# deu439/ARFlow

Hardware: AMD Instinct MI355X
Metric: image-pairs/sec fwd+bwd, PWCLite 384x640 bs=8 (higher is better)
Workload: dtype f32; 1 GPU; pwclite_uflow+uflow_loss, 384x640 pairs, batch 8 per GPU, fwd(both directions)+loss+bwd+allreduce+Adam; global_batch=8, parallelism=dp1, step_start=seeded weights + fresh Adam state, restored before every step, loss_finite=True

## Files before the change

arflow_amd/csrc/splitbf16.hpp:

```cpp
#pragma once
#include <array>

#include "common.hpp"

namespace splitbf16 {
typedef __bf16 bf16x8 __attribute__((ext_vector_type(8)));
typedef float f32x16 __attribute__((ext_vector_type(16)));

struct Split {
  __bf16 p[3];
  __device__ __forceinline__ explicit Split(float v) {
    p[0] = (__bf16)v;
    const float r1 = v - (float)p[0];
    p[1] = (__bf16)r1;
    p[2] = (__bf16)(r1 - (float)p[1]);
  }
};

template <class F>
__device__ __forceinline__ void split8(const F& value, bf16x8 (&o)[3]) {
#pragma unroll
  for (int e = 0; e < 8; ++e) {
    const Split s(value(e));
    o[0][e] = s.p[0], o[1][e] = s.p[1], o[2][e] = s.p[2];
  }
}

__device__ __forceinline__ int acc_channel(int i, int hh) { return (i & 3) + 8 * (i >> 2) + 4 * hh; }

__device__ __forceinline__ void acc_zero(f32x16& a) {
#pragma unroll
  for (int i = 0; i < 16; ++i) a[i] = 0.f;
}
template <class T, int N>
__device__ __forceinline__ void acc_zero(T (&a)[N]) {
#pragma unroll
  for (int s = 0; s < N; ++s) acc_zero(a[s]);
}

inline int tiles32(int n) { return (n + 31) / 32; }
constexpr int MAX_KT = 2;

struct TilePart { int kt, count, first; };
inline std::array<TilePart, 2> split_tiles(int nkt, int max_kt) {
  const int chunks = (nkt + max_kt - 1) / max_kt, base = nkt / chunks, extra = nkt % chunks;
  return {{{base + 1, extra, 0}, {base, chunks - extra, extra * (base + 1)}}};
}

template <auto KERNEL>
inline int allow_dynamic_lds(int bytes) {
  static bool attr_set = false;
  if (!attr_set) {
    const hipError_t e = hipFuncSetAttribute(reinterpret_cast<const void*>(KERNEL), hipFuncAttributeMaxDynamicSharedMemorySize, bytes);
    if (e != hipSuccess) return af_hip_status(e);
    attr_set = true;
  }
  return ARFLOW_OK;
}
}
```

arflow_amd/csrc/splitconv_wgrad.hip:

```cpp
#include <climits>
#include <cstdint>

#include "splitbf16.hpp"

namespace {
using namespace splitbf16;
typedef unsigned u32x4 __attribute__((ext_vector_type(4)));

constexpr int G = 8;
constexpr int DY_CS = 3 * G + 1;
constexpr int X_CS = 9 * G + 1;
constexpr int XH_CS = 9 * G + 1;
constexpr int MAX_ROWS = 128;
constexpr int MIN_ROWS = 4;
constexpr int WANT_WG = 1024;

template <int KT>
struct Lds {
  static constexpr int DY = 0;
  static constexpr int X = KT * 32 * DY_CS * 16;
  static constexpr int XH = X + 32 * X_CS * 16;
  static constexpr int BYTES = XH + 32 * XH_CS * 4;
};

__device__ __forceinline__ unsigned bf16_bits(__bf16 b) { return (unsigned)__builtin_bit_cast(unsigned short, b); }

struct Run {
  float4 a, b;
  float l, r;
};
template <bool VEC>
__device__ __forceinline__ void load_run(const float* __restrict__ row, int col0, int W, bool valid, Run& o) {
  const float4 z = make_float4(0.f, 0.f, 0.f, 0.f);
  if (VEC) {
    const bool in0 = col0 < W, in1 = col0 + 4 < W;
    const float4 t0 = *reinterpret_cast<const float4*>(row + (in0 ? col0 : 0));
    const float4 t1 = *reinterpret_cast<const float4*>(row + (in1 ? col0 + 4 : 0));
    o.a = valid && in0 ? t0 : z;
    o.b = valid && in1 ? t1 : z;
  } else {
    float t[8];
#pragma unroll
    for (int e = 0; e < 8; ++e) t[e] = row[min(col0 + e, W - 1)];
#pragma unroll
    for (int e = 0; e < 8; ++e) t[e] = (valid && col0 + e < W) ? t[e] : 0.f;
    o.a = make_float4(t[0], t[1], t[2], t[3]);
    o.b = make_float4(t[4], t[5], t[6], t[7]);
  }
}

struct Plan {
  int GW, SG, nstrips, RPC, nrb, nct, nkt, kchunks;
  long chunks;
};
inline bool shape_ok(int N, int C, int K, int H, int W) {
  return N > 0 && C > 0 && K > 0 && H > 0 && W > 0 && (long)N * C * H * W <= INT_MAX && (long)N * K * H * W <= INT_MAX &&
         (long)9 * K * C <= INT_MAX;
}
inline Plan make_plan(int N, int C, int K, int H, int W) {
  Plan p;
  p.GW = (W + 7) / 8;
  const int ns = (p.GW + G - 1) / G;
  p.SG = 2 * ((p.GW + 2 * ns - 1) / (2 * ns));
  p.nstrips = (p.GW + p.SG - 1) / p.SG;
  p.nct = tiles32(C), p.nkt = tiles32(K), p.kchunks = (p.nkt + MAX_KT - 1) / MAX_KT;
  const long units = (long)p.nct * p.kchunks * N * p.nstrips;
  const long want = (WANT_WG + units - 1) / units;
  int rpc = (int)((H + want - 1) / want);
  if (rpc < MIN_ROWS) rpc = MIN_ROWS;
  if (rpc > MAX_ROWS) rpc = MAX_ROWS;
  if (rpc > H) rpc = H;
  p.RPC = rpc;
  p.nrb = (H + rpc - 1) / rpc;
  p.chunks = (long)N * p.nstrips * p.nrb;
  return p;
}

template <int KT, bool VEC>
__global__ __launch_bounds__(192 * KT, VEC && KT == 2 ? 3 : 2) void splitconv_wgrad_kernel(const float* __restrict__ x, long x_bs,
                                                                             const float* __restrict__ dy, long dy_bs,
                                                                             float* __restrict__ ws, int C, int K, int H, int W,
                                                                             int kt_first, int kcnt, int nct, int nstrips, int SG,
                                                                             int nrb, int RPC) {
  constexpr int NT = 192 * KT;
  using L = Lds<KT>;
  extern __shared__ __align__(16) unsigned char lds[];
  unsigned* const xh = reinterpret_cast<unsigned*>(lds + L::XH);
  const int tid = threadIdx.x, lane = tid & 63, wv = __builtin_amdgcn_readfirstlane(tid >> 6);
  const int r32 = lane & 31, hh = lane >> 5;
  const int ktl = wv / 3, tr = wv - 3 * ktl;
  const int b = blockIdx.x;
  const int ct = b % nct, kc = (b / nct) % kcnt, chunk = b / (nct * kcnt);
  const int rb = chunk % nrb, strip = (chunk / nrb) % nstrips, n = chunk / (nrb * nstrips);
  const int kt0 = kt_first + kc * KT;
  const int h0 = rb * RPC, h1 = min(H, h0 + RPC);
  const int GW = (W + 7) >> 3, g0 = strip * SG, gcount = min(SG, GW - g0), nsteps = (gcount + 1) >> 1;
  const long HWl = (long)H * W;
  const float* const xn = x + (long)n * x_bs;
  const float* const dyn = dy + (long)n * dy_bs;

  constexpr int NX = 32 * G, NITEM = NX + KT * 32 * G, NSLOT = (NITEM + NT - 1) / NT;
  Run pf[NSLOT];
  const auto fetch = [&](int yx, int ydy) __attribute__((always_inline)) {
#pragma unroll
    for (int j = 0; j < NSLOT; ++j) {
      const int i = tid + j * NT;
      if (i < NX) {
        const int cl = i / G, g = i - cl * G;
        const int c = ct * 32 + cl, col0 = (g0 + g) * 8;
        const bool valid = yx >= 0 && yx < H && c < C && g < gcount;
        const float* row = xn + (valid ? (long)c * HWl + (long)yx * W : 0);
        load_run<VEC>(row, col0, W, valid, pf[j]);
        const float vl = row[max(col0 - 1, 0)], vr = row[min(col0 + 8, W - 1)];
        pf[j].l = (valid && col0 > 0) ? vl : 0.f;
        pf[j].r = (valid && col0 + 8 < W) ? vr : 0.f;
      } else if (i < NITEM && ydy >= 0) {
        const int kl = (i - NX) / G, g = (i - NX) - kl * G;
        const int k = kt0 * 32 + kl, col0 = (g0 + g) * 8;
        const bool valid = k < K && g < gcount;
        const float* row = dyn + (valid ? (long)k * HWl + (long)ydy * W : 0);
        load_run<VEC>(row, col0, W, valid, pf[j]);
      }
    }
  };
  const auto commit = [&](int yx, int ydy) __attribute__((always_inline)) {
    const int slot = (yx + 3) % 3;
#pragma unroll
    for (int j = 0; j < NSLOT; ++j) {
      const int i = tid + j * NT;
      if (i < NX) {
        const int cl = i / G, g = i - cl * G;
        const float v[8] = {pf[j].a.x, pf[j].a.y, pf[j].a.z, pf[j].a.w, pf[j].b.x, pf[j].b.y, pf[j].b.z, pf[j].b.w};
        bf16x8 o[3];
#pragma unroll
        for (int e = 0; e < 8; ++e) {
          const Split s(v[e]);
          o[0][e] = s.p[0], o[1][e] = s.p[1], o[2][e] = s.p[2];
        }
        const Split sl(pf[j].l), sr(pf[j].r);
#pragma unroll
        for (int p = 0; p < 3; ++p) {
          const int at = (slot * 3 + p) * G + g;
          *reinterpret_cast<bf16x8*>(lds + L::X + (cl * X_CS + at) * 16) = o[p];
          xh[cl * XH_CS + at] = (bf16_bits(sl.p[p]) << 16) | bf16_bits(sr.p[p]);
        }
      } else if (i < NITEM && ydy >= 0) {
        const int kl = (i - NX) / G, g = (i - NX) - kl * G;
        const float v[8] = {pf[j].a.x, pf[j].a.y, pf[j].a.z, pf[j].a.w, pf[j].b.x, pf[j].b.y, pf[j].b.z, pf[j].b.w};
        bf16x8 o[3];
#pragma unroll
        for (int e = 0; e < 8; ++e) {
          const Split s(v[e]);
          o[0][e] = s.p[0], o[1][e] = s.p[1], o[2][e] = s.p[2];
        }
#pragma unroll
        for (int p = 0; p < 3; ++p) *reinterpret_cast<bf16x8*>(lds + L::DY + (kl * DY_CS + p * G + g) * 16) = o[p];
      }
    }
  };

  f32x16 tot[3];
  acc_zero(tot);

  const unsigned char* const a_base = lds + L::DY + ((ktl * 32 + r32) * DY_CS + hh) * 16;
  fetch(h0 - 1, -1);
  commit(h0 - 1, -1);
  fetch(h0, -1);
  commit(h0, -1);
  fetch(h0 + 1, h0);
  for (int h = h0; h < h1; ++h) {
    if (h > h0) __syncthreads();
    commit(h + 1, h);
    __syncthreads();
    fetch(h + 2, h + 1 < h1 ? h + 1 : -1);
    const int slot = (h + tr + 2) % 3;
    const unsigned char* const b_base = lds + L::X + (r32 * X_CS + slot * 3 * G + hh) * 16;
    const unsigned* const bh_base = xh + r32 * XH_CS + slot * 3 * G + hh;
    f32x16 acc[3];
    acc_zero(acc);
    const auto x_frags = [&](int p, int t, bf16x8 (&bs)[3]) __attribute__((always_inline)) {
      const u32x4 d = *reinterpret_cast<const u32x4*>(b_base + (p * G + 2 * t) * 16);
      const unsigned nb = bh_base[p * G + 2 * t];
      const unsigned m1 = __builtin_amdgcn_alignbit(d.y, d.x, 16), m2 = __builtin_amdgcn_alignbit(d.z, d.y, 16),
                     m3 = __builtin_amdgcn_alignbit(d.w, d.z, 16);
      const u32x4 lo = {__builtin_amdgcn_alignbit(d.x, nb, 16), m1, m2, m3};
      const u32x4 hi = {m1, m2, m3, __builtin_amdgcn_alignbit(nb, d.w, 16)};
      bs[0] = __builtin_bit_cast(bf16x8, lo);
      bs[1] = __builtin_bit_cast(bf16x8, d);
      bs[2] = __builtin_bit_cast(bf16x8, hi);
    };
#pragma unroll 1
    for (int t = 0; t < nsteps; ++t) {
      bf16x8 a[3], bs[3];
#pragma unroll
      for (int p = 0; p < 3; ++p) a[p] = *reinterpret_cast<const bf16x8*>(a_base + (p * G + 2 * t) * 16);
#pragma unroll
      for (int p = 2; p >= 0; --p) {
        x_frags(p, t, bs);
#pragma unroll
        for (int pa = 2 - p; pa >= (p == 0 ? 1 : 0); --pa)
#pragma unroll
          for (int s = 0; s < 3; ++s) acc[s] = __builtin_amdgcn_mfma_f32_32x32x16_bf16(a[pa], bs[s], acc[s], 0, 0, 0);
      }
    }
#pragma unroll 1
    for (int t = 0; t < nsteps; ++t) {
      bf16x8 bs[3];
      const bf16x8 a0 = *reinterpret_cast<const bf16x8*>(a_base + (2 * t) * 16);
      x_frags(0, t, bs);
#pragma unroll
      for (int s = 0; s < 3; ++s) acc[s] = __builtin_amdgcn_mfma_f32_32x32x16_bf16(a0, bs[s], acc[s], 0, 0, 0);
    }
#pragma unroll
    for (int s = 0; s < 3; ++s) tot[s] = tot[s] + acc[s];
  }
  const int c = ct * 32 + r32;
  if (c < C) {
#pragma unroll
    for (int s = 0; s < 3; ++s) {
      float* const wt = ws + ((long)chunk * 9 + (tr * 3 + s)) * K * C;
#pragma unroll
      for (int i = 0; i < 16; ++i) {
        const int k = 32 * (kt0 + ktl) + acc_channel(i, hh);
        if (k < K) wt[(long)k * C + c] = tot[s][i];
      }
    }
  }
}

__global__ __launch_bounds__(256) void splitconv_wgrad_finish_kernel(const float* __restrict__ ws, float* __restrict__ dw, int K,
                                                                       int C, int chunks) {
  const int KC = K * C, e = blockIdx.x * 256 + threadIdx.x;
  if (e >= 9 * KC) return;
  const int tap = e / KC, kc = e - tap * KC;
  double s = 0.0;
  for (int ch = 0; ch < chunks; ++ch) s += (double)ws[(long)ch * 9 * KC + e];
  dw[(long)kc * 9 + tap] = (float)s;
}

template <int KT, bool VEC>
int launch(const float* x, long x_bs, const float* dy, long dy_bs, float* ws, int C, int K, int H, int W, int kt_first, int kcnt,
           const Plan& p, hipStream_t st) {
  using L = Lds<KT>;
  if (const int rc = allow_dynamic_lds<&splitconv_wgrad_kernel<KT, VEC>>(L::BYTES)) return rc;
  const long grid = p.chunks * kcnt * p.nct;
  if (grid > INT_MAX) return ARFLOW_ESHAPE;
  hipLaunchKernelGGL((splitconv_wgrad_kernel<KT, VEC>), dim3((unsigned)grid), dim3(192 * KT), L::BYTES, st, x, x_bs, dy, dy_bs, ws, C, K,
                     H, W, kt_first, kcnt, p.nct, p.nstrips, p.SG, p.nrb, p.RPC);
  return af_launch_status();
}
}

extern "C" long arflow_splitconv_wgrad_ws_bytes(int N, int C, int K, int H, int W) {
  if (!shape_ok(N, C, K, H, W)) return ARFLOW_ESHAPE;
  const Plan p = make_plan(N, C, K, H, W);
  if (p.chunks > INT_MAX) return ARFLOW_ESHAPE;
  return p.chunks * 9 * K * C * 4;
}

extern "C" int arflow_splitconv_wgrad(const float* x, long x_bstride, const float* dy, long dy_bstride, float* dw, void* ws, int N,
                                      int C, int K, int H, int W, arflow_stream_t stream) {
  af_clear_stale_error();
  AF_REQUIRE_PTR(x);
  AF_REQUIRE_PTR(dy);
  AF_REQUIRE_PTR(dw);
  AF_REQUIRE_PTR(ws);
  AF_REQUIRE(shape_ok(N, C, K, H, W), ARFLOW_ESHAPE);
  AF_REQUIRE(af_stride_ok(x_bstride, N, (long)C * H * W) && af_stride_ok(dy_bstride, N, (long)K * H * W), ARFLOW_ESHAPE);
  AF_REQUIRE(x_bstride >= 0 && dy_bstride >= 0 && x_bstride <= LONG_MAX / N && dy_bstride <= LONG_MAX / N, ARFLOW_ESHAPE);
  AF_REQUIRE((((uintptr_t)x | (uintptr_t)dy | (uintptr_t)dw) & 3) == 0 && af_aligned16(ws), ARFLOW_EPARAM);
  const Plan p = make_plan(N, C, K, H, W);
  AF_REQUIRE(p.chunks <= INT_MAX, ARFLOW_ESHAPE);
  hipStream_t st = (hipStream_t)stream;
  const bool vec = W % 4 == 0 && af_vec4_ok(x, x_bstride, N) && af_vec4_ok(dy, dy_bstride, N);
  for (const TilePart& t : split_tiles(p.nkt, MAX_KT)) {
    if (t.count == 0) continue;
    const auto go = [&](auto kt_c, auto vec_c) {
      return launch<decltype(kt_c)::value, decltype(vec_c)::value>(x, x_bstride, dy, dy_bstride, (float*)ws, C, K, H, W, t.first, t.count, p, st);
    };
    using std::integral_constant;
    const int rc = t.kt == 1 ? (vec ? go(integral_constant<int, 1>{}, std::true_type{}) : go(integral_constant<int, 1>{}, std::false_type{}))
                           : (vec ? go(integral_constant<int, 2>{}, std::true_type{}) : go(integral_constant<int, 2>{}, std::false_type{}));
    if (rc != ARFLOW_OK) return rc;
  }
  hipLaunchKernelGGL(splitconv_wgrad_finish_kernel, dim3((unsigned)af_cdiv((long)9 * K * C, 256)), dim3(256), 0, st,
                     (const float*)ws, dw, K, C, (int)p.chunks);
  return af_launch_status();
}
```

arflow_amd/functional.py:

```python
import contextlib

import torch

from . import _lib
from . import ddp as _ddp

PAD = {'zeros': 0, 'border': 1}
NORM_ARFLOW, NORM_UFLOW = 0, 1


def _need_gpu(*tensors):
    for t in tensors:
        if t is None:
            continue
        if not t.is_cuda:
            raise _lib.ArflowHipError('arflow_amd ops run on the GPU only (got a %s tensor); there is no CPU '
                                      'fallback -- the CPU oracle lives in oracle/ and is test-only' % t.device)
        if t.dtype != torch.float32:
            raise _lib.ArflowHipError('arflow_amd ops are fp32 only (got %s)' % t.dtype)


def _p(t):
    return None if t is None else t.data_ptr()

# ... 371 lines not shown
        return False
    if flow is not None and flow_is_coarse and (H % 2 or W % 2 or tuple(flow.shape[2:]) != (H // 2, W // 2)):
        return False
    return True


_LEVEL_FUSED = __import__('os').environ.get('ARFLOW_LEVEL_FUSED', '1') != '0'


@_samples_mode
class LevelFunction(torch.autograd.Function):

    @staticmethod
    def forward(ctx, x1, x2, flow, cfg, x1_rows, x2_rows, *members):
        _need_gpu(x1, x2, flow, *members)
        if x1.shape != x2.shape or x1.dim() != 4:
            raise ValueError('level expects two [B,C,H,W] feature maps of equal shape')
        x1, x2 = x1.contiguous(), x2.contiguous()
        B, C, H, W = x1.shape
        lib = _lib.load()
        nvol = (2 * cfg.d + 1) ** 2
        has_flow = flow is not None
        chans, offs, off = [], {}, 0
        for item in cfg.layout:
            c = {'vol': nvol, 'x1n': C, 'flow': 2}[item] if isinstance(item, str) else int(members[item].shape[1])
            offs[item] = off
            chans.append(c)
            off += c
        ctot = off
        if 'flow' in offs and not (has_flow and cfg.flow_is_coarse):
            raise ValueError("layout item 'flow' needs a coarse flow")
        buf = torch.empty(B, ctot, H, W, device=x1.device, dtype=torch.float32)
        bs = ctot * H * W
        rows = lib.arflow_level_acc_rows(B, C, H, W, int(has_flow))
        acc = torch.empty(4 * B * rows, device=x1.device, dtype=torch.float64)
        stats = torch.empty(B, 4, device=x1.device, dtype=torch.float32)
        sign = torch.empty(B, 3, H, W, device=x1.device, dtype=torch.int32) if cfg.slope != 1.0 else None
        flow_full = x2w = x1n = None
        fbs, fslot, fup = 0, None, None
        if has_flow:
            flow, fbs = _flow_view(flow)
            x2w = torch.empty_like(x2)
            if cfg.flow_is_coarse:
                flow_full = fup = torch.empty(B, 2, H, W, device=x1.device, dtype=torch.float32)
                fslot = buf[:, offs['flow']:].data_ptr() if 'flow' in offs else None
            else:
                flow_full = flow
        if 'x1n' in offs:
            x1n_ptr, x1n_bs = buf[:, offs['x1n']:].data_ptr(), bs
        else:
            x1n = torch.empty_like(x1)
            x1n_ptr, x1n_bs = x1n.data_ptr(), C * H * W
        for name, rows in (('x1_rows', x1_rows), ('x2_rows', x2_rows)):
            if rows is None:
                continue
            if rows.dtype != torch.float64 or rows.dim() != 3 or rows.shape[0] != B or rows.shape[2] != 2:
                raise ValueError('%s must be [B, rows, 2] float64' % name)
            if rows.device != x1.device:
                raise ValueError('%s must be on the device of the feature maps' % name)
        if x1_rows is not None:
            x1_rows = x1_rows.contiguous()
        if x2_rows is not None:
            x2_rows = x2_rows.contiguous() if (not has_flow and x1_rows is not None) else None
        with torch.cuda.device_of(x1):
            _call('arflow_level_fwd_m', _p(x1), _p(x2), _p(flow), fbs, int(cfg.flow_is_coarse and has_flow), int(cfg.up_align),
                  _p(fup), fslot, bs, _p(x2w), cfg.mode, buf[:, offs['vol']:].data_ptr(), bs, x1n_ptr, x1n_bs, _p(sign),
                  _p(stats), _p(acc), _p(x1_rows), 0 if x1_rows is None else int(x1_rows.shape[1]), _p(x2_rows),
                  0 if x2_rows is None else int(x2_rows.shape[1]), B, C, H, W, cfg.d, cfg.slope, cfg.pad, cfg.align, cfg.norm,
                  _stream(), key=(B, C, H, W, cfg.d, 3 if sign is not None else 0,
                                  int(has_flow) + int(has_flow and cfg.flow_is_coarse), int(x1_rows is not None)))
        for item in cfg.layout:
            if not isinstance(item, str):
                buf[:, offs[item]:offs[item] + int(members[item].shape[1])].copy_(members[item])
        ctx.save_for_backward(x1, x2, x2w, flow_full, stats, sign, buf if x1n is None else x1n)
        ctx.cfg, ctx.offs, ctx.ctot, ctx.n_members, ctx.has_flow = cfg, offs, ctot, len(members), has_flow
        ctx.member_chans = [int(m.shape[1]) for m in members]
        if has_flow and cfg.flow_is_coarse:
            return buf, flow_full
        return buf

    @staticmethod
    def backward(ctx, gbuf, gflow_ext=None):
        x1, x2, x2w, flow_full, stats, sign, x1n_holder = ctx.saved_tensors
        cfg, offs, ctot = ctx.cfg, ctx.offs, ctx.ctot
        B, C, H, W = x1.shape
        nvol = (2 * cfg.d + 1) ** 2
        gbuf = gbuf.contiguous()
        bs = ctot * H * W
        if 'x1n' in offs:
            x1n_ptr, x1n_bs = x1n_holder[:, offs['x1n']:].data_ptr(), bs
        else:
            x1n_ptr, x1n_bs = x1n_holder.data_ptr(), C * H * W
        d1, gx2 = torch.empty_like(x1), torch.empty_like(x1)
        ws = torch.empty(_lib.load().arflow_level_bwd_ws_bytes(B, C, H, W), device=x1.device, dtype=torch.uint8)
        gflow_in = fl = gslot = None
        fbs = 0
        coarse = ctx.has_flow and cfg.flow_is_coarse
        if ctx.has_flow:
            fl, fbs = _flow_view(flow_full)
            gflow_in = torch.empty(B, 2, H // 2, W // 2, device=x1.device, dtype=torch.float32) if coarse else \
                torch.empty(B, 2, H, W, device=x1.device, dtype=torch.float32)
            if 'flow' in offs:
                gslot = gbuf[:, offs['flow']:].data_ptr()
            if gflow_ext is not None:
                gflow_ext = gflow_ext.contiguous()
        gdir = gbuf[:, offs['x1n']:].data_ptr() if 'x1n' in offs else None
        with torch.cuda.device_of(x1):
            _call('arflow_level_bwd', gbuf[:, offs['vol']:].data_ptr(), bs, _p(sign), x1n_ptr, x1n_bs, gdir, bs, _p(x1),
                  _p(x2), _p(x2w), _p(fl), fbs, gslot, bs, _p(gflow_ext), _p(stats), cfg.mode, _p(d1), _p(gx2), _p(gflow_in),
                  int(coarse), int(cfg.up_align), _p(ws), B, C, H, W, cfg.d, cfg.slope, cfg.pad, cfg.align, cfg.norm,
                  _stream(), key=(B, C, H, W, cfg.d, 3 if sign is not None else 0, int(ctx.has_flow) + int(coarse)))
        gm, k = [], 0
        for item in cfg.layout:
            if not isinstance(item, str):
                gm.append((item, gbuf[:, offs[item]:offs[item] + ctx.member_chans[item]]))
        gmembers = [None] * ctx.n_members
        for idx, g in gm:
            gmembers[idx] = g if ctx.needs_input_grad[6 + idx] else None
        return (d1, gx2, gflow_in, None, None, None) + tuple(gmembers)


def level(x1, x2, flow, cfg, *members, x1_rows=None, x2_rows=None):
    return LevelFunction.apply(x1, x2, flow, cfg, x1_rows, x2_rows, *members)


@_samples_mode
class BiasLeakyReLUFunction(torch.autograd.Function):

    @staticmethod
    def forward(ctx, x, bias, slope):
        _need_gpu(x)
        if not x.is_contiguous():
            raise ValueError('bias_leaky_relu expects a contiguous [B,C,...] tensor')
        B, C = x.shape[0], x.shape[1]
        hw = x[0, 0].numel()
        if bias is not None:
            _need_gpu(bias)
            bias = bias.contiguous()
        with torch.cuda.device_of(x):
            _call('arflow_bias_act_fwd', _p(x), _p(bias), _p(x), B, C, hw, float(slope), _stream(), key=(B, C, hw))
        ctx.mark_dirty(x)
        ctx.save_for_backward(x)
        ctx.slope, ctx.has_bias = float(slope), bias is not None
        return x

    @staticmethod
    def backward(ctx, gout):
        y, = ctx.saved_tensors
        B, C = y.shape[0], y.shape[1]
        hw = y[0, 0].numel()
        gout = gout.contiguous()
        gin = torch.empty_like(gout)
        gb = torch.empty(C, device=y.device, dtype=torch.float32) if (ctx.has_bias and ctx.needs_input_grad[1]) else None
        with torch.cuda.device_of(y):
            _call('arflow_bias_act_bwd', _p(gout), _p(y), _p(gin), _p(gb), B, C, hw, ctx.slope, _stream(), key=(B, C, hw))
        return gin, gb, None


def bias_leaky_relu(x, bias, slope=0.1):
    return BiasLeakyReLUFunction.apply(x, bias, slope)


_HEADCONV = __import__('os').environ.get('ARFLOW_HEADCONV', '1') != '0'


class HeadConvFunction(torch.autograd.Function):

    @staticmethod
    def forward(ctx, x, weight, bias):
        _need_gpu(x, weight, bias)
        if x.dim() != 4 or tuple(weight.shape) != (2, x.shape[1], 3, 3):
            raise ValueError('head_conv expects x [B,C,H,W] and weight [2,C,3,3]')
        x, weight = x.contiguous(), weight.contiguous()
        if bias is not None:
            bias = bias.contiguous()
        y = _headconv_fwd(x, weight, bias)
        ctx.save_for_backward(x, weight)
        ctx.has_bias = bias is not None
        return y

    @staticmethod
    def backward(ctx, dy):
        x, weight = ctx.saved_tensors
        dy = dy.contiguous()
        dx = _headconv_dgrad(dy, weight, x) if ctx.needs_input_grad[0] else None
        dw, db = _headconv_wgrad(x, dy, weight, ctx.needs_input_grad[1], ctx.has_bias and ctx.needs_input_grad[2])
        return dx, dw, db


def _headconv_fwd(x, w, b):
    B, C, H, W = x.shape
    y = torch.empty(B, 2, H, W, device=x.device, dtype=torch.float32)
    with torch.cuda.device_of(x):
        _call('arflow_headconv_fwd', _p(x), _p(w), _p(b), _p(y), B, C, H, W, _stream())
    return y


def _headconv_dgrad(gy, w, like):
    B, C, H, W = like.shape
    dx = torch.empty_like(like)
    with torch.cuda.device_of(like):
        _call('arflow_headconv_bwd_data', _p(gy), _p(w), _p(dx), B, C, H, W, _stream())
    return dx


def _headconv_wgrad(x, gy, w, want_w, want_b):
    if not (want_w or want_b):
        return None, None
    B, C, H, W = x.shape
    ws = _workspace('arflow_headconv_bwd_weight_ws_bytes', B, C, H, W, device=x.device)
    dw = torch.empty_like(w)
    db = torch.empty(2, device=x.device, dtype=torch.float32) if want_b else None
    with torch.cuda.device_of(x):
        _call('arflow_headconv_bwd_weight', _p(x), _p(gy), _p(dw), _p(db), _p(ws), B, C, H, W, _stream())
    return (dw if want_w else None), db


def head_conv(x, weight, bias):
    return HeadConvFunction.apply(x, weight, bias)


def head_conv_enabled():
    return _HEADCONV


_SPLITCONV = __import__('os').environ.get('ARFLOW_SPLITCONV', '1') != '0'


def splitconv_enabled():
    return _SPLITCONV


def splitconv_takes(N, C, K, H, W):
    if not _SPLITCONV:
        return False
    return _splitconv_rule(int(N), int(C), int(K), int(H), int(W))


def _size_floor(N, H, W, h, w):
    return H * W >= h * w and N * H * W >= 16 * h * w


def _splitconv_rule(N, C, K, H, W):
    if min(C, K) < 32 or not 64 <= max(C, K) <= 640:
        return False
    if _size_floor(N, H, W, 96, 160):
        return True
    if _size_floor(N, H, W, 48, 80):
        return max(C, K) >= 128 and (K >= 128 or C <= 128)
    return False


def splitconv(x, w, transpose_flip=False, out=None, bias=None, slope=None):
    _need_gpu(x, w, out, bias)
    if x.dim() != 4 or w.dim() != 4 or tuple(w.shape[2:]) != (3, 3) or x.shape[1] != w.shape[0 if transpose_flip else 1]:
        raise ValueError('splitconv expects x [N,C,H,W] and w [K,C,3,3] (transpose_flip: x [N,K,H,W])')
    x, x_bs = _batch_strided(x)
    w = w.contiguous()
    N, C, H, W = x.shape
    K = int(w.shape[1 if transpose_flip else 0])
    if bias is not None and (slope is None or bias.numel() != K):
        raise ValueError('splitconv: bias holds one value per output channel and needs slope (the epilogue is bias + LeakyReLU)')
    packed = _workspace('arflow_splitconv_pack_bytes', K, C, device=x.device)
    if out is None:
        y, y_bs = torch.empty(N, K, H, W, device=x.device, dtype=torch.float32), K * H * W
    else:
        y, y_bs = out, (int(out.stride(0)) if N > 1 else K * H * W)
        if tuple(y.shape) != (N, K, H, W) or _batch_strided(y)[0] is not y:
            raise ValueError('splitconv: out must be an [N,K,H,W] view with dense planes (a channel slot of a larger tensor)')
        if not _disjoint(x, x_bs, y, y_bs):
            raise ValueError('splitconv: out overlaps x')
    bias = None if bias is None else bias.contiguous()
    with torch.cuda.device_of(x):
        _call('arflow_splitconv_pack', _p(w), _p(packed), int(w.shape[0]), int(w.shape[1]), int(bool(transpose_flip)), _stream())
        _call('arflow_splitconv_fwd_ex', _p(x), x_bs, _p(packed), _p(y), y_bs, _p(bias), int(slope is not None),
              float(slope or 0.0), N, C, K, H, W, _stream())
    return y


def _disjoint(x, x_bs, y, y_bs):
    N, hw = x.shape[0], x.shape[2] * x.shape[3]
    cx, cy = x.shape[1] * hw, y.shape[1] * hw
    d = (y.data_ptr() - x.data_ptr()) // 4
    if d >= (N - 1) * x_bs + cx or d + (N - 1) * y_bs + cy <= 0:
        return True
    if x_bs != y_bs:
        return False
    r = d % x_bs
    return r >= cx and r + cy <= x_bs


_SPLITCONV_WGRAD = __import__('os').environ.get('ARFLOW_SPLITCONV_WGRAD', '1') != '0'


def splitconv_wgrad_takes(N, C, K, H, W):
    if not (_SPLITCONV and _SPLITCONV_WGRAD):
        return False
    return _splitconv_wgrad_rule(int(N), int(C), int(K), int(H), int(W))


def _splitconv_wgrad_rule(N, C, K, H, W):
    if N * H * W < 16 * 48 * 80:
        return False
    return _size_floor(N, H, W, 96, 160) and 448 <= C <= 640 and 32 <= K <= 128


def _batch_strided(t):
    _, C, H, W = t.shape
    if t.stride(3) != 1 or t.stride(2) != W or t.stride(1) != H * W or (t.shape[0] > 1 and t.stride(0) < C * H * W):
        t = t.contiguous()
    return t, (int(t.stride(0)) if t.shape[0] > 1 else C * H * W)


def splitconv_wgrad(x, gy):
    _need_gpu(x, gy)
    if x.dim() != 4 or gy.dim() != 4 or x.shape[0] != gy.shape[0] or x.shape[2:] != gy.shape[2:]:
        raise ValueError('splitconv_wgrad expects x [N,C,H,W] and gy [N,K,H,W]')
    x, x_bs = _batch_strided(x)
    gy, gy_bs = _batch_strided(gy)
    N, C, H, W = x.shape
    K = int(gy.shape[1])
    ws = _workspace('arflow_splitconv_wgrad_ws_bytes', N, C, K, H, W, device=x.device)
    dw = torch.empty(K, C, 3, 3, device=x.device, dtype=torch.float32)
    with torch.cuda.device_of(x):
        _call('arflow_splitconv_wgrad', _p(x), x_bs, _p(gy), gy_bs, _p(dw), _p(ws), N, C, K, H, W, _stream())
    return dw


def _conv_args():
    return [1, 1], [1, 1], [1, 1], False, [0, 0], 1


class Conv3x3Function(torch.autograd.Function):

    @staticmethod
    def forward(ctx, x, w, fwd, dgrad, wgrad=False):
        if fwd:
            y = splitconv(x, w)
        else:
            y = torch.ops.aten.convolution(x, w, None, *_conv_args())
        ctx.save_for_backward(x, w)
        ctx.dgrad, ctx.wgrad = bool(dgrad), bool(wgrad)
        return y

    @staticmethod
    @torch.autograd.function.once_differentiable
    def backward(ctx, gy):
        x, w = ctx.saved_tensors
        dx, dw = _conv3x3_grads(x, w, gy.contiguous(), ctx.needs_input_grad[0], ctx.needs_input_grad[1], ctx.dgrad, ctx.wgrad)
        return dx, dw, None, None, None


def _conv3x3_grads(x, w, gy, want_dx, want_dw, dx_native, dw_native):
    dx = splitconv(gy, w, transpose_flip=True) if want_dx and dx_native else None
    dw = splitconv_wgrad(x, gy) if want_dw and dw_native else None
    left = [bool(want_dx and dx is None), bool(want_dw and dw is None), False]
    if any(left):
        dx_m, dw_m, _ = torch.ops.aten.convolution_backward(gy, x, w, None, *_conv_args(), left)
        dx, dw = (dx_m if left[0] else dx), (dw_m if left[1] else dw)
    return dx, dw


def conv3x3(x, w, fwd=True, dgrad=True, wgrad=False):
    return Conv3x3Function.apply(x, w, bool(fwd), bool(dgrad), bool(wgrad))


_DENSE_BLOCK = __import__('os').environ.get('ARFLOW_DENSE_BLOCK', '1') != '0'
DENSE_MAX_SRC = 8


def dense_block_enabled():
    return _DENSE_BLOCK


def _dense_src_type():
    import ctypes

    class DenseSrc(ctypes.Structure):
        _fields_ = [('ptr', ctypes.c_void_p), ('bstride', ctypes.c_long), ('scale', ctypes.c_void_p)]
    return DenseSrc


_DenseSrc = _dense_src_type()


def dense_cat(y, bias, x, slope):
    _need_gpu(y, bias, x)
    if y.dim() != 4 or x.dim() != 4 or y.shape[0] != x.shape[0] or y.shape[2:] != x.shape[2:]:
        raise ValueError('dense_cat expects y [B,oc,H,W] and x [B,C,H,W]')
    y, x = y.contiguous(), x.contiguous()
    bias = None if bias is None else bias.contiguous()
    B, oc, H, W = y.shape
    C = x.shape[1]
    out = torch.empty(B, oc + C, H, W, device=y.device, dtype=torch.float32)
    with torch.cuda.device_of(y):
        _call('arflow_dense_cat_fwd', _p(y), _p(bias), _p(x), _p(out), B, oc, C, H * W, float(slope), _stream(),
              key=(B, oc, C, H * W))
    return out


def dense_grad_gather(sources, oc, act=None, slope=0.1, want_bias=False):
    import ctypes
    if not 1 <= len(sources) <= DENSE_MAX_SRC:
        raise ValueError('dense_grad_gather takes 1..%d sources' % DENSE_MAX_SRC)
    t0 = sources[0][0]
    B, _, H, W = t0.shape
    hw = H * W
    arr = (_DenseSrc * len(sources))()
    keep = []
    for j, (t, off, scale) in enumerate(sources):
        _need_gpu(t, scale)
        st = t.stride()
        if t.dim() != 4 or t.shape[0] != B or tuple(t.shape[2:]) != (H, W) or off < 0 or off + oc > t.shape[1]:
            raise ValueError('dense_grad_gather: source %d does not hold channels %d:%d of a [%d,*,%d,%d] tensor' % (j, off, off + oc, B, H, W))
        if st[3] != 1 or st[2] != W or st[1] != hw:
            t = t.contiguous()
            st = t.stride()
        if scale is not None:
            scale = scale.reshape(-1).contiguous()
            if scale.numel() != B:
                raise ValueError('dense_grad_gather: a scale holds one value per sample')
        keep.append((t, scale))
        arr[j].ptr = t.data_ptr() + 4 * off * hw
        arr[j].bstride = st[0] if B > 1 else t.shape[1] * hw
        arr[j].scale = _p(scale)
    act_bs = 0
    if act is not None:
        _need_gpu(act)
        ok = act.dim() == 4 and act.shape[0] == B and tuple(act.shape[2:]) == (H, W) and act.shape[1] >= oc
        if ok and act.is_contiguous():
            act_bs = act.shape[1] * hw
        elif ok and _batch_strided(act)[0] is act:
            act_bs = int(act.stride(0)) if B > 1 else act.shape[1] * hw
        else:
            raise ValueError('dense_grad_gather: act must be a contiguous [B,>=oc,H,W] tensor')
    gy = torch.empty(B, oc, H, W, device=t0.device, dtype=torch.float32)
    rows = None
    if want_bias:
        n = _lib.load().arflow_dense_gbias_rows(B, hw)
        if n <= 0:
            _lib.check(n, 'arflow_dense_gbias_rows')
        rows = torch.empty(n, oc, device=t0.device, dtype=torch.float32)
    with torch.cuda.device_of(t0):
        _call('arflow_dense_grad_gather', ctypes.cast(arr, ctypes.c_void_p), len(sources), _p(act), act_bs, _p(gy), _p(rows), B,
              oc, hw, float(slope), _stream(), key=(B, oc, hw, len(sources), int(act is not None)))
    return gy, (None if rows is None else rows.sum(0))


_DENSE_INPLACE = __import__('os').environ.get('ARFLOW_DENSE_INPLACE', '1') != '0'


def dense_inplace_enabled():
    return _DENSE_INPLACE


def _inplace_wgrad_takes(N, C, K, H, W):
    if splitconv_wgrad_takes(N, C, K, H, W):
        return True
    return _SPLITCONV and _SPLITCONV_WGRAD and _inplace_wgrad_rule(int(N), int(C), int(K), int(H), int(W))


def _inplace_wgrad_rule(N, C, K, H, W):
    return _size_floor(N, H, W, 96, 160) and 128 <= C < 448 and 96 <= K <= 128


class DenseEstimatorFunction(torch.autograd.Function):

    @staticmethod
    def forward(ctx, x, slope, *params):
        if len(params) != 12:
            raise ValueError('dense_estimator expects (w, b) of five layers and of the head')
        _need_gpu(x, *params)
        slope = float(slope)
        ws, bs = params[0:10:2], params[1:10:2]
        w_head, b_head = params[10], params[11]
        ocs = [int(w.shape[0]) for w in ws]
        B, C1, H, W = x.shape
        cins = [C1 + sum(ocs[:k]) for k in range(5)]
        inplace = _DENSE_INPLACE and all(splitconv_takes(B, c, oc, H, W) for c, oc in zip(cins, ocs))
        if inplace:
            off = sum(ocs)
            x6 = torch.empty(B, C1 + off, H, W, device=x.device, dtype=torch.float32)
            x6[:, off:].copy_(x)
            for w, b, oc in zip(ws, bs, ocs):
                splitconv(x6[:, off:], w, out=x6[:, off - oc:off], bias=b, slope=slope)
                off -= oc
        else:
            xs = [x.contiguous()]
            for w, b in zip(ws, bs):
                xk = xs[-1]
                if splitconv_takes(xk.shape[0], xk.shape[1], w.shape[0], xk.shape[2], xk.shape[3]):
                    y = splitconv(xk, w)
                else:
                    y = torch.nn.functional.conv2d(xk, w, None, 1, 1)
                xs.append(dense_cat(y, b, xk, slope))
            x6 = xs[-1]
        w_head = w_head.contiguous()
        flow = _headconv_fwd(x6, w_head, b_head.contiguous())
        if inplace:
            ctx.save_for_backward(x6, *ws, w_head)
        else:
            ctx.save_for_backward(*xs, *ws, w_head)
        ctx.slope, ctx.inplace = slope, inplace
        ctx.set_materialize_grads(False)
        return x6, flow

    @staticmethod
    @torch.autograd.function.once_differentiable
    def backward(ctx, gx6, gflow):
        if ctx.inplace:
            x6, ws, w_head = ctx.saved_tensors[0], ctx.saved_tensors[1:6], ctx.saved_tensors[6]
            tail = [int(w.shape[0]) for w in ws]
            xs = [x6[:, sum(tail[m:]):] for m in range(5)] + [x6]
        else:
            xs, ws, w_head = ctx.saved_tensors[:6], ctx.saved_tensors[6:11], ctx.saved_tensors[11]
        need = ctx.needs_input_grad
        grads = [None] * 14
        if gx6 is None and gflow is None:
            return tuple(grads)
        x6 = xs[5]
        B, C6, H, W = x6.shape
        ocs = [int(w.shape[0]) for w in ws]
        lowest = 0 if need[0] else next((m for m in range(1, 6) if need[2 * m] or need[2 * m + 1]), 6)
        dx_head = None
        if gflow is not None:
            gflow = gflow.contiguous()
            if lowest < 6:
                dx_head = _headconv_dgrad(gflow, w_head, x6)
            grads[12], grads[13] = _headconv_wgrad(x6, gflow, w_head, need[12], need[13])
        if lowest == 6:
            return tuple(grads)
        top = [t for t in (gx6, dx_head) if t is not None]
        dxs = []
        for m in range(5, max(lowest, 1) - 1, -1):
            srcs = [(t, sum(ocs[m:5]), None) for t in top] + [(dx, sum(ocs[m:k - 1]), None) for dx, k in dxs]
            gy, gb = dense_grad_gather(srcs, ocs[m - 1], act=xs[m], slope=ctx.slope, want_bias=need[2 * m + 1])
            want_dx, want_dw = m > lowest, bool(need[2 * m])
            xm = xs[m - 1]
            dx_native = want_dx and splitconv_takes(B, ocs[m - 1], xm.shape[1], H, W)
            dw_native = want_dw and (_inplace_wgrad_takes if ctx.inplace else splitconv_wgrad_takes)(B, xm.shape[1], ocs[m - 1], H, W)
            dx, dw = _conv3x3_grads(xm, ws[m - 1], gy, want_dx, want_dw, dx_native, dw_native)
            grads[2 * m], grads[2 * m + 1] = dw, gb
            if want_dx:
                dxs.append((dx, m))
        if need[0]:
            srcs = [(t, sum(ocs), None) for t in top] + [(dx, sum(ocs[:k - 1]), None) for dx, k in dxs]
            grads[0] = dense_grad_gather(srcs, int(xs[0].shape[1]))[0]
        return tuple(grads)


def dense_estimator(x, slope, params):
    return DenseEstimatorFunction.apply(x, slope, *params)


@_samples_mode
class BiasLeakyReLUMomentsFunction(torch.autograd.Function):

    @staticmethod
    def forward(ctx, x, bias, slope):
        _need_gpu(x)
        if not x.is_contiguous():
            raise ValueError('bias_leaky_relu expects a contiguous [B,C,...] tensor')
        B, C = x.shape[0], x.shape[1]
        hw = x[0, 0].numel()
        if bias is not None:
            _need_gpu(bias)
            bias = bias.contiguous()
        rows = _lib.load().arflow_bias_act_mom_rows(C, hw)
        mom = torch.empty(B, rows, 2, device=x.device, dtype=torch.float64)
        with torch.cuda.device_of(x):
            _call('arflow_bias_act_fwd_mom', _p(x), _p(bias), _p(x), _p(mom), B, C, hw, float(slope), _stream(), key=(B, C, hw))
        ctx.mark_dirty(x)
        ctx.mark_non_differentiable(mom)
        ctx.save_for_backward(x)
        ctx.slope, ctx.has_bias = float(slope), bias is not None
        return x, mom

    @staticmethod
    def backward(ctx, gout, gmom_unused):
        y, = ctx.saved_tensors
        B, C = y.shape[0], y.shape[1]
        hw = y[0, 0].numel()
        gout = gout.contiguous()
        gin = torch.empty_like(gout)
        gb = torch.empty(C, device=y.device, dtype=torch.float32) if (ctx.has_bias and ctx.needs_input_grad[1]) else None
        with torch.cuda.device_of(y):
            _call('arflow_bias_act_bwd', _p(gout), _p(y), _p(gin), _p(gb), B, C, hw, ctx.slope, _stream(), key=(B, C, hw))
        return gin, gb, None


def bias_leaky_relu_moments(x, bias, slope=0.1):
    return BiasLeakyReLUMomentsFunction.apply(x, bias, slope)


@_samples_mode
class WarpFunction(torch.autograd.Function):

    @staticmethod
    def forward(ctx, src, flow, pad, align_corners, norm, want_valid=False):
        _need_gpu(src, flow)
        src = src.contiguous()
        flow, fbs = _flow_view(flow)
        B, C, Hs, Ws = src.shape
        _, _, H, W = flow.shape
        if flow.shape[0] != B:
            raise ValueError('batch mismatch between source and flow')
        out = torch.empty(B, C, H, W, device=src.device, dtype=torch.float32)
# ... 1072 lines not shown
```

Before: 184.0 image-pairs/s.

## Add two-C-tile wgrad blocks, XCD-aware block remap, and widen splitconv wgrad dispatch

The split-bf16 weight-gradient kernel now lets one workgroup cover up to two 32-channel input tiles alongside two K tiles. The dy rows loaded into LDS are then reused across more input channels. The old per-part launches become a single launch with a block decoder that spreads consecutive blocks across XCDs, and rows-per-chunk is retuned from the CU count. The Python dispatch rule also routes smaller-C and lower-resolution layers to this kernel. Risks include larger workgroups (768 threads) and more LDS per block lowering occupancy, and newly routed shapes possibly running slower than the previous path.

```diff
diff --git a/arflow_amd/csrc/split_tiles.hpp b/arflow_amd/csrc/split_tiles.hpp
--- /dev/null
+++ b/arflow_amd/csrc/split_tiles.hpp
@@ -0,0 +1,13 @@
+#pragma once
+#include <array>
+
+namespace splitbf16 {
+inline int tiles32(int n) { return (n + 31) / 32; }
+constexpr int MAX_KT = 2;
+
+struct TilePart { int kt, count, first; };
+inline std::array<TilePart, 2> split_tiles(int n, int max_t) {
+  const int chunks = (n + max_t - 1) / max_t, base = n / chunks, extra = n % chunks;
+  return {{{base + 1, extra, 0}, {base, chunks - extra, extra * (base + 1)}}};
+}
+}
diff --git a/arflow_amd/csrc/splitbf16.hpp b/arflow_amd/csrc/splitbf16.hpp
--- a/arflow_amd/csrc/splitbf16.hpp
+++ b/arflow_amd/csrc/splitbf16.hpp
@@ -2,6 +2,7 @@
 #include <array>
 
 #include "common.hpp"
+#include "split_tiles.hpp"
 
 namespace splitbf16 {
 typedef __bf16 bf16x8 __attribute__((ext_vector_type(8)));
@@ -38,14 +39,6 @@
   for (int s = 0; s < N; ++s) acc_zero(a[s]);
 }
 
-inline int tiles32(int n) { return (n + 31) / 32; }
-constexpr int MAX_KT = 2;
-
-struct TilePart { int kt, count, first; };
-inline std::array<TilePart, 2> split_tiles(int nkt, int max_kt) {
-  const int chunks = (nkt + max_kt - 1) / max_kt, base = nkt / chunks, extra = nkt % chunks;
-  return {{{base + 1, extra, 0}, {base, chunks - extra, extra * (base + 1)}}};
-}
 
 template <auto KERNEL>
 inline int allow_dynamic_lds(int bytes) {
diff --git a/arflow_amd/csrc/splitconv_wgrad.hip b/arflow_amd/csrc/splitconv_wgrad.hip
--- a/arflow_amd/csrc/splitconv_wgrad.hip
+++ b/arflow_amd/csrc/splitconv_wgrad.hip
@@ -2,25 +2,23 @@
 #include <cstdint>
 
 #include "splitbf16.hpp"
+#include "splitconv_wgrad_plan.hpp"
 
 namespace {
 using namespace splitbf16;
+using namespace wgrad_plan;
 typedef unsigned u32x4 __attribute__((ext_vector_type(4)));
 
-constexpr int G = 8;
 constexpr int DY_CS = 3 * G + 1;
 constexpr int X_CS = 9 * G + 1;
 constexpr int XH_CS = 9 * G + 1;
-constexpr int MAX_ROWS = 128;
-constexpr int MIN_ROWS = 4;
-constexpr int WANT_WG = 1024;
-
-template <int KT>
+
+template <int KT, int CT>
 struct Lds {
   static constexpr int DY = 0;
   static constexpr int X = KT * 32 * DY_CS * 16;
-  static constexpr int XH = X + 32 * X_CS * 16;
-  static constexpr int BYTES = XH + 32 * XH_CS * 4;
+  static constexpr int XH = X + CT * 32 * X_CS * 16;
+  static constexpr int BYTES = XH + CT * 32 * XH_CS * 4;
 };
 
 __device__ __forceinline__ unsigned bf16_bits(__bf16 b) { return (unsigned)__builtin_bit_cast(unsigned short, b); }
@@ -49,57 +47,27 @@
   }
 }
 
-struct Plan {
-  int GW, SG, nstrips, RPC, nrb, nct, nkt, kchunks;
-  long chunks;
-};
-inline bool shape_ok(int N, int C, int K, int H, int W) {
-  return N > 0 && C > 0 && K > 0 && H > 0 && W > 0 && (long)N * C * H * W <= INT_MAX && (long)N * K * H * W <= INT_MAX &&
-         (long)9 * K * C <= INT_MAX;
-}
-inline Plan make_plan(int N, int C, int K, int H, int W) {
-  Plan p;
-  p.GW = (W + 7) / 8;
-  const int ns = (p.GW + G - 1) / G;
-  p.SG = 2 * ((p.GW + 2 * ns - 1) / (2 * ns));
-  p.nstrips = (p.GW + p.SG - 1) / p.SG;
-  p.nct = tiles32(C), p.nkt = tiles32(K), p.kchunks = (p.nkt + MAX_KT - 1) / MAX_KT;
-  const long units = (long)p.nct * p.kchunks * N * p.nstrips;
-  const long want = (WANT_WG + units - 1) / units;
-  int rpc = (int)((H + want - 1) / want);
-  if (rpc < MIN_ROWS) rpc = MIN_ROWS;
-  if (rpc > MAX_ROWS) rpc = MAX_ROWS;
-  if (rpc > H) rpc = H;
-  p.RPC = rpc;
-  p.nrb = (H + rpc - 1) / rpc;
-  p.chunks = (long)N * p.nstrips * p.nrb;
-  return p;
-}
-
-template <int KT, bool VEC>
-__global__ __launch_bounds__(192 * KT, VEC && KT == 2 ? 3 : 2) void splitconv_wgrad_kernel(const float* __restrict__ x, long x_bs,
-                                                                             const float* __restrict__ dy, long dy_bs,
-                                                                             float* __restrict__ ws, int C, int K, int H, int W,
-                                                                             int kt_first, int kcnt, int nct, int nstrips, int SG,
-                                                                             int nrb, int RPC) {
-  constexpr int NT = 192 * KT;
-  using L = Lds<KT>;
+template <int KT, int CT, bool VEC>
+__global__ __launch_bounds__(192 * KT * CT, VEC && KT == 2 ? 3 : 2) void splitconv_wgrad_kernel(
+    const float* __restrict__ x, long x_bs, const float* __restrict__ dy, long dy_bs, float* __restrict__ ws, int C, int K, int H,
+    int W, const Launch l, int SG, int RPC) {
+  constexpr int NT = 192 * KT * CT;
+  using L = Lds<KT, CT>;
   extern __shared__ __align__(16) unsigned char lds[];
   unsigned* const xh = reinterpret_cast<unsigned*>(lds + L::XH);
   const int tid = threadIdx.x, lane = tid & 63, wv = __builtin_amdgcn_readfirstlane(tid >> 6);
   const int r32 = lane & 31, hh = lane >> 5;
-  const int ktl = wv / 3, tr = wv - 3 * ktl;
-  const int b = blockIdx.x;
-  const int ct = b % nct, kc = (b / nct) % kcnt, chunk = b / (nct * kcnt);
-  const int rb = chunk % nrb, strip = (chunk / nrb) % nstrips, n = chunk / (nrb * nstrips);
-  const int kt0 = kt_first + kc * KT;
-  const int h0 = rb * RPC, h1 = min(H, h0 + RPC);
+  const int tile = wv / 3, tr = wv - 3 * tile, ctl = tile / KT, ktl = tile - KT * ctl;
+  const Block blk = decode_block(blockIdx.x, gridDim.x, l);
+  const int chunk = blk.chunk, strip = blk.strip, n = blk.n, kt0 = blk.kt0, ct0 = blk.ct0;
+  const int cend = min(C, (ct0 + blk.ctn) * 32), kend = min(K, (kt0 + blk.ktn) * 32);
+  const int h0 = blk.rb * RPC, h1 = min(H, h0 + RPC);
   const int GW = (W + 7) >> 3, g0 = strip * SG, gcount = min(SG, GW - g0), nsteps = (gcount + 1) >> 1;
   const long HWl = (long)H * W;
   const float* const xn = x + (long)n * x_bs;
   const float* const dyn = dy + (long)n * dy_bs;
 
-  constexpr int NX = 32 * G, NITEM = NX + KT * 32 * G, NSLOT = (NITEM + NT - 1) / NT;
+  constexpr int NX = CT * 32 * G, NITEM = NX + KT * 32 * G, NSLOT = (NITEM + NT - 1) / NT;
   Run pf[NSLOT];
   const auto fetch = [&](int yx, int ydy) __attribute__((always_inline)) {
 #pragma unroll
@@ -107,8 +75,8 @@
       const int i = tid + j * NT;
       if (i < NX) {
         const int cl = i / G, g = i - cl * G;
-        const int c = ct * 32 + cl, col0 = (g0 + g) * 8;
-        const bool valid = yx >= 0 && yx < H && c < C && g < gcount;
+        const int c = ct0 * 32 + cl, col0 = (g0 + g) * 8;
+        const bool valid = yx >= 0 && yx < H && c < cend && g < gcount;
         const float* row = xn + (valid ? (long)c * HWl + (long)yx * W : 0);
         load_run<VEC>(row, col0, W, valid, pf[j]);
         const float vl = row[max(col0 - 1, 0)], vr = row[min(col0 + 8, W - 1)];
@@ -117,7 +85,7 @@
       } else if (i < NITEM && ydy >= 0) {
         const int kl = (i - NX) / G, g = (i - NX) - kl * G;
         const int k = kt0 * 32 + kl, col0 = (g0 + g) * 8;
-        const bool valid = k < K && g < gcount;
+        const bool valid = k < kend && g < gcount;
         const float* row = dyn + (valid ? (long)k * HWl + (long)ydy * W : 0);
         load_run<VEC>(row, col0, W, valid, pf[j]);
       }
@@ -174,8 +142,9 @@
     __syncthreads();
     fetch(h + 2, h + 1 < h1 ? h + 1 : -1);
     const int slot = (h + tr + 2) % 3;
-    const unsigned char* const b_base = lds + L::X + (r32 * X_CS + slot * 3 * G + hh) * 16;
-    const unsigned* const bh_base = xh + r32 * XH_CS + slot * 3 * G + hh;
+    const unsigned char* const b_base = lds + L::X + ((ctl * 32 + r32) * X_CS + slot * 3 * G + hh) * 16;
+    const unsigned* const bh_base = xh + (ctl * 32 + r32) * XH_CS + slot * 3 * G + hh;
+    if (ctl >= blk.ctn || ktl >= blk.ktn) continue;
     f32x16 acc[3];
     acc_zero(acc);
     const auto x_frags = [&](int p, int t, bf16x8 (&bs)[3]) __attribute__((always_inline)) {
@@ -214,15 +183,14 @@
 #pragma unroll
     for (int s = 0; s < 3; ++s) tot[s] = tot[s] + acc[s];
   }
-  const int c = ct * 32 + r32;
-  if (c < C) {
+  const int c = (ct0 + ctl) * 32 + r32;
+  if (c < cend) {
 #pragma unroll
     for (int s = 0; s < 3; ++s) {
-      float* const wt = ws + ((long)chunk * 9 + (tr * 3 + s)) * K * C;
 #pragma unroll
       for (int i = 0; i < 16; ++i) {
         const int k = 32 * (kt0 + ktl) + acc_channel(i, hh);
-        if (k < K) wt[(long)k * C + c] = tot[s][i];
+        if (k < kend) ws[ws_index(chunk, tr * 3 + s, k, c, K, C)] = tot[s][i];
       }
     }
   }
@@ -238,16 +206,19 @@
   dw[(long)kc * 9 + tap] = (float)s;
 }
 
-template <int KT, bool VEC>
-int launch(const float* x, long x_bs, const float* dy, long dy_bs, float* ws, int C, int K, int H, int W, int kt_first, int kcnt,
+template <int KT, int CT, bool VEC>
+int launch(const float* x, long x_bs, const float* dy, long dy_bs, float* ws, int C, int K, int H, int W, const Launch& l,
            const Plan& p, hipStream_t st) {
-  using L = Lds<KT>;
-  if (const int rc = allow_dynamic_lds<&splitconv_wgrad_kernel<KT, VEC>>(L::BYTES)) return rc;
-  const long grid = p.chunks * kcnt * p.nct;
-  if (grid > INT_MAX) return ARFLOW_ESHAPE;
-  hipLaunchKernelGGL((splitconv_wgrad_kernel<KT, VEC>), dim3((unsigned)grid), dim3(192 * KT), L::BYTES, st, x, x_bs, dy, dy_bs, ws, C, K,
-                     H, W, kt_first, kcnt, p.nct, p.nstrips, p.SG, p.nrb, p.RPC);
-  return af_launch_status();
+  if constexpr (CT > plan_ct(KT, VEC)) {
+    return ARFLOW_ESHAPE;
+  } else {
+    using L = Lds<KT, CT>;
+    if (const int rc = allow_dynamic_lds<&splitconv_wgrad_kernel<KT, CT, VEC>>(L::BYTES)) return rc;
+    if (l.blocks > INT_MAX) return ARFLOW_ESHAPE;
+    hipLaunchKernelGGL((splitconv_wgrad_kernel<KT, CT, VEC>), dim3((unsigned)l.blocks), dim3(192 * KT * CT), L::BYTES, st, x, x_bs, dy,
+                       dy_bs, ws, C, K, H, W, l, p.SG, p.RPC);
+    return af_launch_status();
+  }
 }
 }
 
@@ -255,7 +226,7 @@
   if (!shape_ok(N, C, K, H, W)) return ARFLOW_ESHAPE;
   const Plan p = make_plan(N, C, K, H, W);
   if (p.chunks > INT_MAX) return ARFLOW_ESHAPE;
-  return p.chunks * 9 * K * C * 4;
+  return ws_bytes(p, K, C);
 }
 
 extern "C" int arflow_splitconv_wgrad(const float* x, long x_bstride, const float* dy, long dy_bstride, float* dw, void* ws, int N,
@@ -273,16 +244,18 @@
   AF_REQUIRE(p.chunks <= INT_MAX, ARFLOW_ESHAPE);
   hipStream_t st = (hipStream_t)stream;
   const bool vec = W % 4 == 0 && af_vec4_ok(x, x_bstride, N) && af_vec4_ok(dy, dy_bstride, N);
-  for (const TilePart& t : split_tiles(p.nkt, MAX_KT)) {
-    if (t.count == 0) continue;
-    const auto go = [&](auto kt_c, auto vec_c) {
-      return launch<decltype(kt_c)::value, decltype(vec_c)::value>(x, x_bstride, dy, dy_bstride, (float*)ws, C, K, H, W, t.first, t.count, p, st);
-    };
-    using std::integral_constant;
-    const int rc = t.kt == 1 ? (vec ? go(integral_constant<int, 1>{}, std::true_type{}) : go(integral_constant<int, 1>{}, std::false_type{}))
-                           : (vec ? go(integral_constant<int, 2>{}, std::true_type{}) : go(integral_constant<int, 2>{}, std::false_type{}));
-    if (rc != ARFLOW_OK) return rc;
-  }
+  const Launch l = make_launch(p, vec);
+  const auto go = [&](auto kt_c, auto ct_c, auto vec_c) {
+    return launch<decltype(kt_c)::value, decltype(ct_c)::value, decltype(vec_c)::value>(x, x_bstride, dy, dy_bstride, (float*)ws, C, K, H,
+                                                                                        W, l, p, st);
+  };
+  const auto go_ct = [&](auto kt_c, auto vec_c) {
+    return l.ct == 1 ? go(kt_c, std::integral_constant<int, 1>{}, vec_c) : go(kt_c, std::integral_constant<int, 2>{}, vec_c);
+  };
+  const auto go_kt = [&](auto vec_c) {
+    return l.kt == 1 ? go_ct(std::integral_constant<int, 1>{}, vec_c) : go_ct(std::integral_constant<int, 2>{}, vec_c);
+  };
+  if (const int rc = vec ? go_kt(std::true_type{}) : go_kt(std::false_type{})) return rc;
   hipLaunchKernelGGL(splitconv_wgrad_finish_kernel, dim3((unsigned)af_cdiv((long)9 * K * C, 256)), dim3(256), 0, st,
                      (const float*)ws, dw, K, C, (int)p.chunks);
   return af_launch_status();
diff --git a/arflow_amd/csrc/splitconv_wgrad_plan.hpp b/arflow_amd/csrc/splitconv_wgrad_plan.hpp
--- /dev/null
+++ b/arflow_amd/csrc/splitconv_wgrad_plan.hpp
@@ -0,0 +1,96 @@
+#pragma once
+#include <climits>
+
+#include "split_tiles.hpp"
+
+#if defined(__HIPCC__)
+#define WGRAD_HD __host__ __device__
+#else
+#define WGRAD_HD
+#endif
+
+namespace wgrad_plan {
+using splitbf16::MAX_KT;
+using splitbf16::split_tiles;
+using splitbf16::tiles32;
+
+constexpr int G = 8;
+constexpr int MAX_CT = 2;
+constexpr int MAX_ROWS = 128;
+constexpr int MIN_ROWS = 4;
+constexpr int NCU = 256;
+constexpr int NXCD = 8;
+
+struct Plan {
+  int GW, SG, nstrips, RPC, nrb, nct, nkt;
+  int kt, kchunks;
+  long chunks;
+};
+inline bool shape_ok(int N, int C, int K, int H, int W) {
+  return N > 0 && C > 0 && K > 0 && H > 0 && W > 0 && (long)N * C * H * W <= INT_MAX && (long)N * K * H * W <= INT_MAX &&
+         (long)9 * K * C <= INT_MAX;
+}
+constexpr int plan_ct(int kt, bool vec) { return kt == MAX_KT && vec ? MAX_CT : 1; }
+inline Plan make_plan(int N, int C, int K, int H, int W) {
+  Plan p;
+  p.GW = (W + 7) / 8;
+  const int ns = (p.GW + G - 1) / G;
+  p.SG = 2 * ((p.GW + 2 * ns - 1) / (2 * ns));
+  p.nstrips = (p.GW + p.SG - 1) / p.SG;
+  p.nct = tiles32(C), p.nkt = tiles32(K);
+  p.kt = p.nkt < MAX_KT ? p.nkt : MAX_KT, p.kchunks = (p.nkt + MAX_KT - 1) / MAX_KT;
+  const int ct = plan_ct(p.kt, true);
+  const long units = (long)((p.nct + ct - 1) / ct) * p.kchunks * N * p.nstrips;
+  const long want_wg = 2 * NCU * (ct == MAX_CT ? 1 : 2);
+  const long want = (want_wg + units - 1) / units;
+  int rpc = (int)((H + want - 1) / want);
+  if (rpc < MIN_ROWS) rpc = MIN_ROWS;
+  if (rpc > MAX_ROWS) rpc = MAX_ROWS;
+  if (rpc > H) rpc = H;
+  p.RPC = rpc;
+  p.nrb = (H + rpc - 1) / rpc;
+  p.chunks = (long)N * p.nstrips * p.nrb;
+  return p;
+}
+inline long ws_bytes(const Plan& p, int K, int C) { return p.chunks * 9 * K * C * 4; }
+
+struct Launch {
+  int kt, kparts, kbase, kextra;
+  int ct, cparts, cbase, cextra;
+  int nstrips, nrb;
+  long blocks;
+};
+inline Launch make_launch(const Plan& p, bool vec) {
+  Launch l;
+  const auto k = split_tiles(p.nkt, MAX_KT), c = split_tiles(p.nct, plan_ct(p.kt, vec));
+  l.kt = p.kt, l.kparts = k[0].count + k[1].count, l.kbase = k[1].kt, l.kextra = k[0].count;
+  l.ct = c[0].count ? c[0].kt : c[1].kt, l.cparts = c[0].count + c[1].count, l.cbase = c[1].kt, l.cextra = c[0].count;
+  l.nstrips = p.nstrips, l.nrb = p.nrb;
+  l.blocks = p.chunks * l.kparts * l.cparts;
+  return l;
+}
+
+WGRAD_HD inline unsigned xcd_remap(unsigned orig, unsigned nwg) {
+  const unsigned q = nwg / NXCD, r = nwg % NXCD, x = orig % NXCD;
+  return (x < r ? x * (q + 1) : r * (q + 1) + (x - r) * q) + orig / NXCD;
+}
+
+struct Block {
+  int n, strip, rb, chunk;
+  int kt0, ktn;
+  int ct0, ctn;
+};
+WGRAD_HD inline Block decode_block(unsigned block_id, unsigned nwg, const Launch& l) {
+  const int b = (int)xcd_remap(block_id, nwg);
+  const int cp = b % l.cparts, kp = (b / l.cparts) % l.kparts;
+  Block o;
+  o.chunk = b / (l.cparts * l.kparts);
+  o.rb = o.chunk % l.nrb, o.strip = (o.chunk / l.nrb) % l.nstrips, o.n = o.chunk / (l.nrb * l.nstrips);
+  o.kt0 = kp < l.kextra ? kp * (l.kbase + 1) : l.kextra * (l.kbase + 1) + (kp - l.kextra) * l.kbase;
+  o.ktn = kp < l.kextra ? l.kbase + 1 : l.kbase;
+  o.ct0 = cp < l.cextra ? cp * (l.cbase + 1) : l.cextra * (l.cbase + 1) + (cp - l.cextra) * l.cbase;
+  o.ctn = cp < l.cextra ? l.cbase + 1 : l.cbase;
+  return o;
+}
+WGRAD_HD inline long ws_index(int chunk, int tap, int k, int c, int K, int C) { return (((long)chunk * 9 + tap) * K + k) * C + c; }
+}
diff --git a/arflow_amd/functional.py b/arflow_amd/functional.py
--- a/arflow_amd/functional.py
+++ b/arflow_amd/functional.py
@@ -697,7 +697,9 @@
 def _splitconv_wgrad_rule(N, C, K, H, W):
     if N * H * W < 16 * 48 * 80:
         return False
-    return _size_floor(N, H, W, 96, 160) and 448 <= C <= 640 and 32 <= K <= 128
+    if _size_floor(N, H, W, 96, 160):
+        return 128 <= C <= 640 and 32 <= K <= 128
+    return H * W < 96 * 160 and _size_floor(N, H, W, 48, 80) and 256 <= C <= 640 and 64 <= K <= 128
 
 
 def _batch_strided(t):
```

After: 195.1 image-pairs/s, median of 6. 1.06x the previous value.
